# joeylitalien/drmlt-mitsuba

Measured on AMD Instinct MI355X. Metric: mutations/sec (accepted+rejected), higher is better.
Workload: dtype f32

## Files before the change

### drmlt-mitsuba_amd/csrc/device_sampler.h

```cpp
#pragma once
#include "device_math.h"
#include "device_types.h"

extern __shared__ __attribute__((aligned(16))) float lds_x[];

#define FP_STRICT _Pragma("clang fp contract(off)")

DEV float load_global_f32(const float *p) { return *(const float __attribute__((address_space(1))) *) (uintptr_t) p; }

enum { SM_BOOT = 0, SM_ARRAY = 1, SM_STAGE1 = 2, SM_STAGE2 = 3, SM_REVERSE = 4, SM_PT = 5 };

DEV float wrap01(float y) { return y > 1.f ? 2.f - y : fabsf(y); }
DEV float unwrap01(float v) { return v < 0.f ? 2.f - v : (v > 1.f ? -v : v); }

#define KELEMEN_S1 (1.0f / 1024.0f)
#define KELEMEN_S2 (1.0f / 64.0f)
#define ORBITAL_SCALE 1.9f
#define LOG2_S1_OVER_S2 (-4.0f)
#define WC_DISPERSION 0.96954361f

DEV float kelemen_sample(float xi, float s2) {
        FP_STRICT;
    float sign = 1.f;
    if (xi < 0.5f) { xi *= 2.f; } else { sign = -1.f; xi = 2.f * (xi - 0.5f); }
// ... 91 lines not shown
    uint32_t lane;
    uint32_t u1_off, s2_off;
    uint32_t stride;

    DEV void reset_caches() {}
    DEV float x(uint32_t k) const { return lds_x[k * stride + lane]; }
    DEV float u1(uint32_t k) const { return lds_x[u1_off + k * stride + lane]; }
    DEV float s2(uint32_t k) const { return lds_x[s2_off + k * stride + lane]; }
    DEV void put4(uint32_t off, const Unit4 &u) const {
        float *dst = &lds_x[off + lane];
        dst[0] = u.v[0]; dst[stride] = u.v[1]; dst[2u * stride] = u.v[2]; dst[3u * stride] = u.v[3];
    }

    DEV void fill_stage1(uint32_t b0, uint32_t b1) {
        for (uint32_t b = b0; b < b1; ++b) put4(u1_off + b * 4u * stride, philox_unit4(key0, key1, b, major, chain, TAG_S1));
    }
    DEV void fill_stage2(uint32_t D4, uint32_t first, uint32_t step) {
        if (large || type == 2) {
            const uint32_t rows = large ? D4 : (D4 / 2u + 3u) & ~3u;
            for (uint32_t b = first; b < rows / 4u; b += step) put4(s2_off + b * 4u * stride, philox_unit4(key0, key1, b, major, chain, TAG_S2));
        } else {
            for (uint32_t b = first; b < D4 / 2u; b += step) {
                const Unit4 u = philox_unit4(key0, key1, b, major, chain, TAG_S2);
                float *dst = &lds_x[s2_off + b * 2u * stride + lane];
                dst[0] = gaussian_sample(u.v[0], u.v[1], sigma2);
                dst[stride] = gaussian_sample(u.v[2], u.v[3], sigma2);
            }
        }
    }

    DEV float y_raw(uint32_t k) const {
        if (large) return u1(k);
        if (type != 2) return iid_first(u1(k), x(k));
        const uint32_t k0 = k & ~1u;
        return orbital_first(u1(k0), u1(k0 + 1u), (k & 1u) != 0u, x(k));
    }
    DEV float z_raw(uint32_t k) const {
        if (large) return s2(k);
        if (type != 2) return iid_second(x(k), s2(k));
        float z0, z1;
        orbital_pair(k & ~1u, true, z0, z1);
        return (k & 1u) ? z1 : z0;
    }
    DEV float next(uint32_t k) const {
        if (type == 2 && mode == SM_STAGE1) {
            const uint32_t k0 = k & ~1u;
            const bool odd = (k & 1u) != 0u;
            const float ua = u1(k0), ub = u1(k0 + 1u);
            const float y = orbital_first(ua, ub, odd, x(k));
            return wrap01(large ? (odd ? ub : ua) : y);
        }
        if (type == 2) {
            float z0, z1;
            orbital_pair(k & ~1u, true, z0, z1);
            const float zl = s2(k);
            return wrap01(large ? zl : ((k & 1u) ? z1 : z0));
        }
        const float xk = x(k), a = u1(k), g = s2(k);
        const float y = large ? a : iid_first(a, xk);
        const float z = large ? g : iid_second(xk, g);
        const float v = mode == SM_STAGE1 ? y : (mode == SM_STAGE2 ? z : green_reverse(xk, y, z));
        return wrap01(v);
    }
    DEV void orbital_pair(uint32_t k0, bool second, float &o0, float &o1) const {
        const float x0 = x(k0), x1 = x(k0 + 1u);
        float y0, y1;
        orbital_first_pair(u1(k0), u1(k0 + 1u), x0, x1, y0, y1);
        if (!second) { o0 = y0; o1 = y1; return; }
        orbital_second_pair(s2(k0 >> 1), x0, x1, y0, y1, o0, o1);
    }
};

template <int RULE = RULE_GENERIC> struct RowSamplerT {
    static constexpr bool orbital = RULE == RULE_ORBITAL;
    static constexpr bool batch_draws = true;
    uint32_t key0, key1;
    int mode, type;
    float sigma2;
    uint32_t stride, x_off, y_off, xyz;

    DEV void reset_caches() {}
    DEV float x(uint32_t k) const { return wrap01(lds_x[x_off + k * stride]); }
    DEV float y_raw(uint32_t k) const { return lds_x[y_off + k * stride]; }
    DEV uint32_t z_off() const { return xyz - x_off - y_off; }
    DEV float z_raw(uint32_t k) const { return lds_x[z_off() + k * stride]; }
    DEV float next(uint32_t k) const {
        if constexpr (orbital) return wrap01(lds_x[(mode == SM_STAGE1 ? y_off : z_off()) + k * stride]);
        float v = y_raw(k);
        if (mode != SM_STAGE1) {
            const float z = z_raw(k);
            v = mode == SM_STAGE2 ? z : green_reverse(x(k), v, z);
        }
        return wrap01(v);
    }
    DEV void adopt(int commit_mode) {
        const uint32_t xo = x_off, zo = z_off();
        x_off = commit_mode == SM_STAGE1 ? y_off : (commit_mode == SM_STAGE2 ? zo : xo);
        y_off = commit_mode == SM_STAGE1 ? xo : y_off;
    }
    DEV uint32_t roles() const { return (x_off << 1) | (y_off << 16); }
    DEV void set_roles(uint32_t w, uint32_t group, uint32_t col) { x_off = (w >> 1) & 0x7fffu; y_off = w >> 16; xyz = 3u * (group + col); }
    DEV static uint32_t first_roles(uint32_t group, uint32_t col) { return (col << 1) | ((group + col) << 16); }
    DEV void fill_first(uint32_t b, uint32_t major, uint32_t chain, bool large) const {
        const Unit4 u = philox_unit4(key0, key1, b, major, chain, TAG_S1);
        const float *xs = &lds_x[x_off + 4u * b * stride];
        float *ys = &lds_x[y_off + 4u * b * stride];
        const float x4[4] = {wrap01(xs[0]), wrap01(xs[stride]), wrap01(xs[2u * stride]), wrap01(xs[3u * stride])};
        float y[4];
        first_stage_block(orbital ? 2 : type, large, u, x4, y);
        ys[0] = y[0]; ys[stride] = y[1]; ys[2u * stride] = y[2]; ys[3u * stride] = y[3];
    }
    DEV void fill_second(uint32_t b, uint32_t D4, uint32_t major, uint32_t chain, bool large) const {
        const uint32_t nblk = large ? D4 / 4u : ((orbital || type == 2) ? (D4 / 2u + 3u) / 4u : D4 / 2u);
        if (b >= nblk) return;
        const Unit4 u = philox_unit4(key0, key1, b, major, chain, TAG_S2);
        const uint32_t zo = z_off();
        if (large) {
#pragma unroll
            for (uint32_t i = 0; i < 4u; ++i) lds_x[zo + (4u * b + i) * stride] = u.v[i];
        } else if (orbital || type == 2) {
            float xa[4], xb[4], ya[4], yb[4];
#pragma unroll
            for (uint32_t i = 0; i < 4u; ++i) {
                const uint32_t k0 = 2u * (4u * b + i), kk = k0 + 1u < D4 ? k0 : 0u;
                xa[i] = x(kk); xb[i] = x(kk + 1u);
                ya[i] = y_raw(kk); yb[i] = y_raw(kk + 1u);
            }
#pragma unroll
            for (uint32_t i = 0; i < 4u; ++i) {
                const uint32_t k0 = 2u * (4u * b + i);
                if (k0 + 1u < D4) {
                    float z0, z1;
                    orbital_second_pair(u.v[i], xa[i], xb[i], ya[i], yb[i], z0, z1);
                    lds_x[zo + k0 * stride] = z0;
                    lds_x[zo + (k0 + 1u) * stride] = z1;
                }
            }
        } else {
            const uint32_t k = 2u * b;
            const float x0 = x(k), x1 = x(k + 1u);
            lds_x[zo + k * stride] = iid_second(u.v[0], u.v[1], sigma2, x0);
            lds_x[zo + (k + 1u) * stride] = iid_second(u.v[2], u.v[3], sigma2, x1);
        }
    }
};
typedef RowSamplerT<> RowSampler;
template <int RULE> DEV void row_fill_first_drawn(const RowSamplerT<RULE> &s, uint32_t b, const Unit4 &u, bool large) {
    const float *xs = &lds_x[s.x_off + 4u * b * s.stride];
    float *ys = &lds_x[s.y_off + 4u * b * s.stride];
    const float x4[4] = {wrap01(xs[0]), wrap01(xs[s.stride]), wrap01(xs[2u * s.stride]), wrap01(xs[3u * s.stride])};
    float y[4];
    first_stage_block(RowSamplerT<RULE>::orbital ? 2 : s.type, large, u, x4, y);
    ys[0] = y[0]; ys[s.stride] = y[1]; ys[2u * s.stride] = y[2]; ys[3u * s.stride] = y[3];
}

struct RowsLds {
    DEV float get(uint32_t k, uint32_t col) const { return lds_x[k * 64u + col]; }
    DEV void put(uint32_t k, uint32_t col, float v) const { lds_x[k * 64u + col] = v; }
};
struct RowsMem {
    typedef float __attribute__((address_space(1))) *GPtr;
    GPtr base;
    uint32_t stride;
    DEV float get(uint32_t k, uint32_t col) const { return base[(size_t) k * stride + col]; }
    DEV void put(uint32_t k, uint32_t col, float v) const { base[(size_t) k * stride + col] = v; }
};

template <class Rows> struct PoolRowSampler {
    static constexpr bool batch_draws = true;
    uint32_t lane;
    Rows rows;
    const float *mira_x = nullptr;
    size_t mira_stride = 0;
    uint32_t mira_k0 = 0u, mira_k1 = 0u, mira_major = 0u, mira_chain = 0u, cached = 0xffffffffu;
    u4 blk = {0u, 0u, 0u, 0u};
    DEV void reset_caches() { cached = 0xffffffffu; }
    DEV float row(uint32_t k) const { return rows.get(k, lane); }
    DEV float next(uint32_t k) const { return wrap01(row(k)); }
    DEV float x(uint32_t k) const { return load_global_f32(mira_x + (size_t) k * mira_stride); }
    DEV float y_raw(uint32_t k) {
        if (cached != (k >> 2)) { cached = k >> 2; blk = philox4x32_10(mira_k0, mira_k1, cached, mira_major, mira_chain, TAG_S1); }
        uint32_t bx = blk.x, by = blk.y, bz = blk.z, bw = blk.w;
        asm volatile("" : "+v"(bx), "+v"(by), "+v"(bz), "+v"(bw));
        const uint32_t c = k & 3u, w = (c & 2u) ? ((c & 1u) ? bw : bz) : ((c & 1u) ? by : bx);
        return iid_first(u32_to_unit(w), x(k));
    }
    DEV float z_raw(uint32_t k) const { return row(k); }
};

struct State4 { float x0, x1, x2, x3; };
DEV State4 v5_state4(const DParams &P, uint32_t D, size_t xcol, uint32_t b) {
    const bool hi = 4u * b + 2u < D;
    const float *xs = P.x + (size_t) (4u * b) * P.n_chains + xcol;
    State4 X;
    X.x0 = load_global_f32(xs); X.x1 = load_global_f32(xs + P.n_chains);
    X.x2 = load_global_f32(xs + (hi ? 2u : 0u) * (size_t) P.n_chains); X.x3 = load_global_f32(xs + (hi ? 3u : 1u) * (size_t) P.n_chains);
    return X;
}
template <class Rows> DEV void v5_fill_first(const DParams &P, const Rows &rows, uint32_t D, uint32_t col, const State4 &X, uint32_t b, uint32_t major, uint32_t chain, bool large) {
    const Unit4 u = philox_unit4(P.key0, P.key1, b, major, chain, TAG_S1);
    const float u0 = u.v[0], u1 = u.v[1], u2 = u.v[2], u3 = u.v[3];
    const bool hi = 4u * b + 2u < D;
    const float x0 = X.x0, x1 = X.x1, x2 = X.x2, x3 = X.x3;
    float y0, y1, y2, y3;
    if (P.type == 2) {
        orbital_first_pair(u0, u1, x0, x1, y0, y1);
        orbital_first_pair(u2, u3, x2, x3, y2, y3);
    } else {
        y0 = iid_first(u0, x0); y1 = iid_first(u1, x1);
        y2 = iid_first(u2, x2); y3 = iid_first(u3, x3);
    }
    rows.put(4u * b, col, large ? u0 : y0); rows.put(4u * b + 1u, col, large ? u1 : y1);
    if (hi) { rows.put(4u * b + 2u, col, large ? u2 : y2); rows.put(4u * b + 3u, col, large ? u3 : y3); }
}
template <class Rows> DEV void v5_fill_second(const DParams &P, const Rows &rows, uint32_t D, uint32_t col, size_t xcol, uint32_t b, uint32_t major, uint32_t chain, bool large) {
    const Unit4 u = philox_unit4(P.key0, P.key1, b, major, chain, TAG_S2);
    if (large) {
#pragma unroll
        for (uint32_t i = 0; i < 4u; ++i)
            if (4u * b + i < D) rows.put(4u * b + i, col, u.v[i]);
        return;
    }
    if (P.type != 2) {
        const uint32_t k = 2u * b;
        const float x0 = load_global_f32(P.x + (size_t) k * P.n_chains + xcol), x1 = load_global_f32(P.x + (size_t) (k + 1u) * P.n_chains + xcol);
        rows.put(k, col, iid_second(u.v[0], u.v[1], P.sigma2, x0));
        rows.put(k + 1u, col, iid_second(u.v[2], u.v[3], P.sigma2, x1));
        return;
    }
    float xa[4], xb[4], ya[4], yb[4];
#pragma unroll
    for (uint32_t i = 0; i < 4u; ++i) {
        const uint32_t k0 = 2u * (4u * b + i);
        const uint32_t kk = k0 + 1u < D ? k0 : 0u;
        xa[i] = load_global_f32(P.x + (size_t) kk * P.n_chains + xcol); xb[i] = load_global_f32(P.x + (size_t) (kk + 1u) * P.n_chains + xcol);
        ya[i] = rows.get(kk, col); yb[i] = rows.get(kk + 1u, col);
    }
#pragma unroll
    for (uint32_t i = 0; i < 4u; ++i) {
        const uint32_t k0 = 2u * (4u * b + i);
        if (k0 + 1u < D) {
            float z0, z1;
            orbital_second_pair(u.v[i], xa[i], xb[i], ya[i], yb[i], z0, z1);
            rows.put(k0, col, z0);
            rows.put(k0 + 1u, col, z1);
        }
    }
}
template <class Rows> DEV void v5_iid_second_again(const DParams &P, const Rows &rows, uint32_t D, uint32_t col, size_t xcol, uint32_t b, uint32_t major, uint32_t chain, bool large, bool reverse) {
    const Unit4 u2 = philox_unit4(P.key0, P.key1, b, major, chain, TAG_S2);
    if (large) {
        Unit4 u1 = u2;
        if (reverse) u1 = philox_unit4(P.key0, P.key1, b, major, chain, TAG_S1);
#pragma unroll
        for (uint32_t i = 0; i < 4u; ++i) {
            const uint32_t k = 4u * b + i;
            if (k < D) {
                float *xg = P.x + (size_t) k * P.n_chains + xcol;
                if (reverse) rows.put(k, col, green_reverse(load_global_f32(xg), u1.v[i], u2.v[i]));
                else *xg = wrap01(u2.v[i]);
            }
        }
        return;
    }
    const uint32_t k = 2u * b;
    float *xg0 = P.x + (size_t) k * P.n_chains + xcol, *xg1 = xg0 + P.n_chains;
    const float x0 = load_global_f32(xg0), x1 = load_global_f32(xg1);
    const float z0 = iid_second(u2.v[0], u2.v[1], P.sigma2, x0), z1 = iid_second(u2.v[2], u2.v[3], P.sigma2, x1);
    if (!reverse) { *xg0 = wrap01(z0); *xg1 = wrap01(z1); return; }
    const u4 r1 = philox4x32_10(P.key0, P.key1, k >> 2, major, chain, TAG_S1);
    const float ua = (k & 2u) ? u32_to_unit(r1.z) : u32_to_unit(r1.x), ub = (k & 2u) ? u32_to_unit(r1.w) : u32_to_unit(r1.y);
    const float y0 = iid_first(ua, x0), y1 = iid_first(ub, x1);
    rows.put(k, col, green_reverse(x0, y0, z0));
    rows.put(k + 1u, col, green_reverse(x1, y1, z1));
}

struct PssmltSampler {
    uint32_t key0, key1, chain, major;
    bool large, kelemen;
    float sigma;
    uint32_t lane;
    uint32_t n_exist;
    u4 b1;
    uint32_t b1_idx;
    DEV void reset_caches() { b1_idx = 0xffffffffu; }
    DEV float u_s1(uint32_t idx) {
        uint32_t blk = idx >> 2;
        if (blk != b1_idx) { b1 = philox4x32_10(key0, key1, blk, major, chain, TAG_S1); b1_idx = blk; }
        return pick4(b1, idx & 3u);
    }
    DEV float x(uint32_t k) const { return lds_x[k * 64u + lane]; }
    DEV float next(uint32_t k) {
        const uint32_t per = (large || kelemen) ? 1u : 2u;
        if (k >= n_exist) return u_s1(per * n_exist + (k - n_exist));
        if (large) return u_s1(k);
        float value = x(k);
        if (kelemen) {
            float xi = u_s1(k);
            const bool add = xi < 0.5f;
            xi = add ? 2.f * xi : 2.f * (xi - 0.5f);
            const float dv = KELEMEN_S2 * fast_exp2(xi * LOG2_S1_OVER_S2);
            if (add) { value += dv; if (value > 1.f) value -= 1.f; }
            else { value -= dv; if (value < 0.f) value += 1.f; }
            return value;
        }
        const float v = value + gaussian_sample(u_s1(2u * k), u_s1(2u * k + 1u), sigma);
// ... 4 lines not shown
```

### drmlt-mitsuba_amd/csrc/kernels.hip

```cpp
#include <algorithm>
#include <cstdlib>
#include <cstdio>
#include <type_traits>
#include "device_path.h"

#include "kernel_common.h"
#include "launch_plan.h"

__device__ __attribute__((noinline)) DSplat eval_boot_sample(const DParams &P, uint32_t index, uint32_t &nd) {
    Sampler smp;
    smp.key0 = P.key0; smp.key1 = P.key1; smp.chain = P.boot_stream; smp.major = index;
    smp.mode = SM_BOOT; smp.arr = nullptr;
    uint32_t nr;
    return eval_path(P, smp, nr, nd);
}

__global__ void __launch_bounds__(64) k_bootstrap(DParams P, uint32_t n, float *lum_out) {
    uint32_t i = blockIdx.x * blockDim.x + threadIdx.x;
    if (i >= n) return;
    uint32_t nd;
    DSplat s = eval_boot_sample(P, i, nd);
    lum_out[i] = s.lum;
    if (P.boot_weighted) { normalize_splat(s, P); lum_out[(size_t) n + i] = s.lum; }
}
// ... 890 lines not shown
    G.z0 = v[8]; G.z1 = v[9]; G.z2 = v[10]; G.z3 = v[11];
}
DEV W2HeldScene w2_held_scene(const DParams &P) {
    W2HeldScene H;
    const uint32_t n_box = (uint32_t) min(max(P.n_box, 0), 3), n_flat = (uint32_t) min(max(P.n_flat_rec, 0), 1);
#pragma unroll
    for (uint32_t i = 0; i < 3u; ++i) {
        BoxRec &G = H.S.box[i];
        const DPrimBox *q = P.prims_box + i;
        w2_hold_rows(G, q->c, q->rz, i < n_box);
        uint32_t f0 = 0u, f1 = 0u, f2 = 0u;
        if (i < n_box) { f0 = q->fw[0]; f1 = q->fw[1]; f2 = q->fw[2]; }
        hold_v(f0); hold_v(f1); hold_v(f2);
        G.f0 = f0; G.f1 = f1; G.f2 = f2;
    }
    FlatRec &F = H.S.flat;
    w2_hold_rows(F, P.prims_flat->c, P.prims_flat->rz, n_flat > 0u);
    int ks = -1;
    if (n_flat > 0u) ks = P.prims_flat->kind_shade;
    hold_v(ks);
    F.ks = ks;
    H.counts = n_box | (n_flat << 8);
    hold_v(H.counts);
    return H;
}

template <bool HELD> __global__ void __launch_bounds__(CHAIN_BLOCK, 2) k_mutate_w2(DParams P, uint32_t n_mut, uint32_t mut_base) {
    typedef RowSamplerT<RULE_ORBITAL> RowSampler;
    if (threadIdx.x == 0) {
        atomicAdd(P.stats + 14, 1ull); atomicAdd(P.stats + 15, 1ull); atomicAdd(P.stats + 16, 1ull);
        if constexpr (HELD) atomicAdd(P.stats + 17, 1ull);
    }
    const uint32_t lane = threadIdx.x;
    const uint32_t sub = lane & 31u;
    const bool helper = lane >= 32u;
    const uint32_t c = blockIdx.x * 32u + sub;
    const bool live = !helper && c < P.n_chains;
    const uint32_t cc = c < P.n_chains ? c : P.n_chains - 1;
    const uint32_t S = V4_STRIDE;
    int smp_mode = SM_STAGE1;
    uint32_t roles;
    uint32_t qn = 0u;
    ChainState cs;
    float cum = 0.f;
    Counters ct = {0u, 0u, 0u, 0u, 0u};
    PathState ps;
    bool helper_has_ray = false;
    Hit h{-1, 0.f, 0.f, 0.f};
    int batch;
    uint32_t base = 0u, target = 0u, limit = 0u;
    bool reported = false;
    W2Held held = w2_held(P);
    w2_hold(held);
    typename std::conditional<HELD, W2HeldScene, W2StreamedScene>::type scene;
    if constexpr (HELD) scene = w2_held_scene(P);
    uint32_t imp_lo = (uint32_t) (uintptr_t) P.importance, imp_hi = (uint32_t) ((uintptr_t) P.importance >> 32);
    uint32_t done_lo = (uint32_t) (uintptr_t) P.chain_done, done_hi = (uint32_t) ((uintptr_t) P.chain_done >> 32);
    uint32_t left_lo = (uint32_t) (uintptr_t) P.waves_left, left_hi = (uint32_t) ((uintptr_t) P.waves_left >> 32);
    uint32_t key0_v = P.key0, key1_v = P.key1, chain_off_v = P.chain_offset, timid_v = (uint32_t) P.timid_after_large;
    hold_v(imp_lo); hold_v(imp_hi); hold_v(done_lo); hold_v(done_hi); hold_v(left_lo); hold_v(left_hi);
    hold_v(key0_v); hold_v(key1_v); hold_v(chain_off_v); hold_v(timid_v);
    {
        const V4Layout<RULE_ORBITAL> Y = v4_layout<RULE_ORBITAL>(P, V4_QCAP);
        roles = RowSampler::first_roles(Y.group, sub);
        if (!helper) {
            for (uint32_t k = 0; k < Y.D; ++k) lds_x[k * S + sub] = unwrap01(P.x[(size_t) k * P.n_chains + cc]);
            for (uint32_t k = Y.D; k < Y.D4; ++k) lds_x[k * S + sub] = 0.f;
        }
        cs.cur.lum = P.cur_lum[cc]; cs.cur.px = P.cur_px[cc]; cs.cur.py = P.cur_py[cc];
        cs.cur.r = P.cur_r[cc]; cs.cur.g = P.cur_g[cc]; cs.cur.b = P.cur_b[cc];
        cs.y = cs.cur; cs.z = cs.cur;
        cs.a1 = 0.f; cs.coin_acc1 = cs.coin_acc2 = cs.coin_mix = 0.f;
        cs.it = 0u; cs.nd1 = cs.nd2 = 0u; cs.stage = -1; cs.large = false;
        path_init(P, ps);
        base = (P.chain_done && live) ? P.chain_done[cc] : mut_base;
        target = P.chain_done ? n_mut : mut_base + n_mut;
        limit = P.chain_done ? P.run_limit : target;
        ps.phase = (live && base < limit) ? PH_DONE : PH_IDLE;
        ps.o = mk3(0.f, 0.f, 0.f); ps.d = mk3(0.f, 0.f, 1.f); ps.tmin = 0.f; ps.tmax = 0.f;
        batch = P.mh_batch > 32 ? 32 : P.mh_batch;
        stage_tables(P, Y.LT, lane);
        if (!helper) {
            const u4 coins = philox4x32_10(P.key0, P.key1, 0u, base, P.chain_offset + blockIdx.x * 32u + sub, TAG_COIN);
            float *dst = &lds_x[Y.L.coin_off + sub];
            dst[0] = u32_to_unit(coins.x); dst[S] = u32_to_unit(coins.y); dst[2u * S] = u32_to_unit(coins.z); dst[3u * S] = u32_to_unit(coins.w);
        }
    }

    for (;;) {
        const bool parked = ps.phase == PH_DONE;
        const unsigned long long pmask = __ballot(parked);
        const unsigned long long rmask = __ballot(ps.phase != PH_DONE && ps.phase != PH_IDLE);
        if (!pmask && !rmask) break;
        if (pmask && (__popcll(pmask) >= batch || !rmask)) {
            DParams Pm{};
            Pm.importance = uniform_ptr<const float>(imp_lo, imp_hi); Pm.width = (int) wave_uniform((uint32_t) held.width); Pm.height = (int) wave_uniform((uint32_t) held.height);
            Pm.chain_done = uniform_ptr<uint32_t>(done_lo, done_hi); Pm.waves_left = uniform_ptr<uint32_t>(left_lo, left_hi);
            Pm.key0 = wave_uniform(key0_v); Pm.key1 = wave_uniform(key1_v); Pm.chain_offset = wave_uniform(chain_off_v);
            Pm.eff_dim = (int) wave_uniform((uint32_t) held.eff_dim); Pm.timid_after_large = (int) wave_uniform(timid_v);
            Pm.use_mixture = 0; Pm.acceptance_map = 0; Pm.type = 2;
            const W2Held &C = held;
            const V4Lds L{C.coin_off, C.list_off, C.q_off, C.qcap};
            RowSampler smp = w2_sampler(Pm.key0, Pm.key1);
            smp.set_roles(roles, C.group, sub); smp.mode = smp_mode;
            const uint32_t D4 = ((uint32_t) Pm.eff_dim + 3u) & ~3u, nb1 = D4 / 4u;
            int *const lds_list = reinterpret_cast<int *>(&lds_x[L.list_off]);
            __builtin_amdgcn_s_setprio(2);
            if (qn + 64u > wave_uniform(L.qcap)) { SECTION_PARAMS(Pf); w2_flush(Pf, L, qn, lane); }
            int commit = 0, kind = 0;
            W2hQueued qa{false, 0.f, 0.f, 0.f, 0.f, 0.f}, qb{false, 0.f, 0.f, 0.f, 0.f, 0.f};
            if constexpr (HELD) w2h_decide(Pm, parked, cs, ps, ct, cum, commit, kind, qa, qb);
            else if (parked) {
                const MhDigest o = mh_decide<RULE_ORBITAL>(Pm, cs, smp, ps, ct);
                if (o.decided) {
                    cum += o.w.w0;
                    const bool a1st = o.acc1, a2nd = o.acc2, adopt = a1st || a2nd;
                    const DSplat sb = select_splat(a2nd, cs.y, cs.z);
                    const float wb = a2nd ? o.w.w1 : o.w.w2;
                    qb.want = !a1st && wb > 0.f;
                    qb.px = sb.px; qb.py = sb.py; qb.r = sb.r * wb; qb.g = sb.g * wb; qb.b = sb.b * wb;
                    const DSplat sa = select_splat(adopt, cs.cur, cs.y);
                    const float wa = adopt ? cum : o.w.w1;
                    qa.want = wa > 0.f;
                    qa.px = sa.px; qa.py = sa.py; qa.r = sa.r * wa; qa.g = sa.g * wa; qa.b = sa.b * wa;
                    if (adopt) {
                        cum = a1st ? o.w.w1 : o.w.w2;
                        cs.cur = select_splat(a1st, cs.y, cs.z);
                    }
                    commit = mh_commit_mode(o);
                }
                kind = cs.stage < 0 ? 4 : 2;
            }
            kind = mh_resolve_kind(Pm, kind, live, base + cs.it, target, limit, reported, lane);
            v4_enqueue(L, qn, qa.want, qa.px, qa.py, qa.r, qa.g, qa.b);
            v4_enqueue(L, qn, qb.want, qb.px, qb.py, qb.r, qb.g, qb.b);


            smp.adopt(commit);
            roles = smp.roles();

            if (parked && kind == 1) {
                const float *cn = &lds_x[L.coin_off + sub];
                cs.large = cn[0] < C.p_large;
                cs.coin_acc1 = cn[S]; cs.coin_acc2 = cn[2u * S]; cs.coin_mix = cn[3u * S];
                cs.stage = 0;
                cs.nd1 = cs.nd2 = 0u;
            }

            RowSampler smg = w2_sampler(Pm.key0, Pm.key1);
            const uint32_t chain_base_g = Pm.chain_offset + blockIdx.x * 32u;
            const uint32_t maj_mine = base + cs.it;
            const unsigned info = roles | (cs.large ? 1u : 0u);
            const uint32_t f1mask = (uint32_t) __ballot(kind == 1);
            if (f1mask) {
                if (kind == 1) lds_list[__builtin_amdgcn_mbcnt_lo(f1mask, 0u)] = (int) sub;
                const uint32_t n = (uint32_t) __popc(f1mask), total = n * (nb1 + 1u);
                const float rcp_n = 1.f / (float) n;
                for (uint32_t fb = 0u; fb < total; fb += 64u) {
                    const uint32_t i = fb + lane;
                    const bool valid = i < total;
                    const uint32_t ii = valid ? i : 0u;
                    const uint32_t b = (uint32_t) (((float) ii + 0.5f) * rcp_n), j = ii - b * n;
                    const uint32_t cj = (uint32_t) lds_list[j];
                    const uint32_t mj = (uint32_t) __shfl((int) maj_mine, (int) cj, 64);
                    const unsigned inf = (unsigned) __shfl((int) info, (int) cj, 64);
                    smg.set_roles(inf, C.group, cj);
                    const bool coin = b >= nb1;
                    if (valid) {
                        const u4 r = philox4x32_10(Pm.key0, Pm.key1, coin ? 0u : b, coin ? mj + 1u : mj, chain_base_g + cj, coin ? TAG_COIN : TAG_S1);
                        const Unit4 u{{u32_to_unit(r.x), u32_to_unit(r.y), u32_to_unit(r.z), u32_to_unit(r.w)}};
                        if (!coin) row_fill_first_drawn(smg, b, u, (inf & 1u) != 0u);
                        else {
                            float *dst = &lds_x[L.coin_off + cj];
                            dst[0] = u.v[0]; dst[S] = u.v[1]; dst[2u * S] = u.v[2]; dst[3u * S] = u.v[3];
                        }
                    }
                }
            }
            const uint32_t f2mask = (uint32_t) __ballot(kind == 2);
            if (f2mask) {
                if (kind == 2) lds_list[__builtin_amdgcn_mbcnt_lo(f2mask, 0u)] = (int) sub;
                const uint32_t nb2 = Pm.timid_after_large ? D4 / 4u : (D4 / 2u + 3u) / 4u;
                const uint32_t n = (uint32_t) __popc(f2mask), total = n * nb2;
                const float rcp_n = 1.f / (float) n;
                for (uint32_t fb = 0u; fb < total; fb += 64u) {
                    const uint32_t i = fb + lane;
                    const bool valid = i < total;
                    const uint32_t ii = valid ? i : 0u;
                    const uint32_t b = (uint32_t) (((float) ii + 0.5f) * rcp_n), j = ii - b * n;
                    const uint32_t cj = (uint32_t) lds_list[j];
                    const uint32_t mj = (uint32_t) __shfl((int) maj_mine, (int) cj, 64);
                    const unsigned inf = (unsigned) __shfl((int) info, (int) cj, 64);
                    smg.set_roles(inf, C.group, cj);
                    if (valid) smg.fill_second(b, D4, mj, chain_base_g + cj, (inf & 1u) != 0u);
                }
            }

            if (parked) {
                if (kind == 0) ps.phase = PH_IDLE;
                else {
                    DParams Vb{};
                    Vb.exclude_direct = C.exclude_direct; Vb.width = C.width; Vb.height = C.height;
                    Vb.tan_half_fov = C.tan_half_fov; Vb.inv_aspect = C.inv_aspect; Vb.near_clip = C.near_clip; Vb.far_clip = C.far_clip;
#pragma unroll
                    for (int q = 0; q < 12; ++q) Vb.cam[q] = C.cam[q];
                    smp_mode = smp.mode = cs.stage == 0 ? SM_STAGE1 : SM_STAGE2;
                    path_init(Vb, ps);
                    const float v0 = smp.next(0u), v1 = smp.next(1u);
                    path_begin(Vb, ps, v0, v1);
                }
            }
        }
        const bool tracing = helper ? helper_has_ray : ps.phase == PH_CLOSEST;
        __builtin_amdgcn_s_setprio(0);
        if constexpr (HELD) {
            if (__ballot(tracing)) {
                const uint32_t counts = wave_uniform(scene.counts);
                h = trace_held(scene.S, counts & 0xffu, counts >> 8, ps.o, ps.d, ps.tmin, ps.tmax);
            }
        } else {
            SECTION_PARAMS(Pt);
            if (__ballot(tracing)) h = trace<0>(Pt, ps.o, ps.d, ps.tmin, ps.tmax, helper);
        }
        __builtin_amdgcn_s_setprio(3);
        const unsigned occluded = from_upper_u((helper_has_ray && h.prim >= 0) ? 1u : 0u);
        helper_has_ray = false;
        ShadowRay sr;
        asm volatile("" : "=v"(sr.d.x), "=v"(sr.d.y), "=v"(sr.d.z), "=v"(sr.tmin), "=v"(sr.tmax));
        sr.o = ps.o; sr.valid = false;
        {
            const W2Held &Cs = held;
            if (!helper && ps.phase != PH_DONE && ps.phase != PH_IDLE) {
                RowSampler sms = w2_sampler(0u, 0u);
                sms.set_roles(roles, Cs.group, sub); sms.mode = smp_mode;
                DParams Vs{};
                Vs.eff_dim = Cs.eff_dim; Vs.rr_depth = Cs.rr_depth; Vs.max_depth = Cs.max_depth;
                const LdsTables LT{Cs.shade_off, Cs.bsdf_off, 0u};
                path_step_diffuse<RowSampler, HeldLightTables, false, HELD>(Vs, HeldLightTables{LT, Cs.light, Cs.light_shade}, ps, sms, h, occluded == 0u, sr);
            }
        }
        ps.o.x = lower_keeps(ps.o.x, sr.o.x); ps.o.y = lower_keeps(ps.o.y, sr.o.y); ps.o.z = lower_keeps(ps.o.z, sr.o.z);
        ps.d.x = lower_keeps(ps.d.x, sr.d.x); ps.d.y = lower_keeps(ps.d.y, sr.d.y); ps.d.z = lower_keeps(ps.d.z, sr.d.z);
        ps.tmin = lower_keeps(ps.tmin, sr.tmin); ps.tmax = lower_keeps(ps.tmax, sr.tmax);
        helper_has_ray = lower_keeps_u(0u, sr.valid ? 1u : 0u) != 0u;
    }
    SECTION_PARAMS(Pe);
    const V4Layout<RULE_ORBITAL> Y = v4_layout<RULE_ORBITAL>(Pe, V4_QCAP);
    if (qn + 32u > Y.L.qcap) w2_flush(Pe, Y.L, qn, lane);
    v4_enqueue(Y.L, qn, live && cum > 0.f, cs.cur.px, cs.cur.py, cs.cur.r * cum, cs.cur.g * cum, cs.cur.b * cum);
    w2_flush(Pe, Y.L, qn, lane);
    if (live) {
        RowSampler smp = Y.smp;
        smp.set_roles(roles, Y.group, sub);
        for (uint32_t k = 0; k < Y.D; ++k) Pe.x[(size_t) k * Pe.n_chains + c] = smp.x(k);
        Pe.cur_lum[c] = cs.cur.lum; Pe.cur_px[c] = cs.cur.px; Pe.cur_py[c] = cs.cur.py;
        Pe.cur_r[c] = cs.cur.r; Pe.cur_g[c] = cs.cur.g; Pe.cur_b[c] = cs.cur.b;
        if (Pe.chain_done) Pe.chain_done[c] = base + cs.it;
    }
    if (Pe.chain_done && !reported && lane == 0) atomicSub(Pe.waves_left, 1u);
    flush_counters(Pe, ct, lane);
    const unsigned long long decided = wave_sum((live && !helper) ? cs.it : 0u);
    if (lane == 0) atomicAdd(Pe.stats + 9, decided);
}

#define V5_STACK32_CAP 25
#ifndef V5_ROWS_MEM_WAVES
#define V5_ROWS_MEM_WAVES 3
#endif
#ifndef V5_ROWS_MEM_STACK32_CAP
#define V5_ROWS_MEM_STACK32_CAP 25
#endif
enum { RS_IDLE = 0, RS_BUSY = 1, RS_DONE = 2 };

struct V5Lds {
    uint32_t coin_off, list_off;
    uint32_t q_off;
    uint32_t pool_off;
    uint32_t ring_off;
    uint32_t status_off;
};
DEV V5Lds v5_layout(uint32_t D, uint32_t qcap, bool coin_rows) {
    V5Lds L;
    L.coin_off = D * 64u;
    L.list_off = L.coin_off + (coin_rows ? 4u * 64u : 0u);
    L.q_off = L.list_off + 64u;
    L.pool_off = L.q_off + 5u * qcap;
    L.ring_off = L.pool_off + 8u * V5_SLOTS;
    L.status_off = L.ring_off + V5_SLOTS / 4u;
    return L;
}

template <int FEAT, bool STACK16, bool OVF, bool STAMPS = false, bool LDS_TABLES = false, bool ROWS_MEM = false>
__global__ void __launch_bounds__(CHAIN_BLOCK, ROWS_MEM ? V5_ROWS_MEM_WAVES : 2) k_mutate_v5(DParams P, uint32_t n_mut, uint32_t mut_base) {
    constexpr bool FLAT = (FEAT & 8) == 0;
    typedef typename std::conditional<ROWS_MEM, RowsMem, RowsLds>::type RowsT;
    typedef PoolRowSampler<RowsT> SamplerT;
    constexpr uint32_t QCAP = (FLAT || STACK16) ? V5_QCAP : V5_QCAP_STACK32;
    constexpr bool COIN_ROWS = FLAT || STACK16;
    SECTION_PARAMS(P0);
    const uint32_t lane = threadIdx.x;
    const uint32_t wave_base = blockIdx.x * 64u;
    const uint32_t c = wave_base + lane;
    const bool live = c < P0.n_chains;
    const uint32_t cc = live ? c : P0.n_chains - 1;
    const uint32_t D = (uint32_t) P0.eff_dim, nb1 = (D + 3u) / 4u;
    const V5Lds L = v5_layout(ROWS_MEM ? 0u : D, QCAP, COIN_ROWS);
    const V4Lds Lq{0u, 0u, L.q_off, QCAP};
    unsigned char *const ring = reinterpret_cast<unsigned char *>(&lds_x[L.ring_off]);
    unsigned char *const status = reinterpret_cast<unsigned char *>(&lds_x[L.status_off]);
    int *const lds_list = reinterpret_cast<int *>(&lds_x[L.list_off]);
    float *const pool = &lds_x[L.pool_off];
    status[lane] = RS_IDLE; status[64u + lane] = RS_IDLE;
    LdsTables LT;
    LT.shade_off = L.status_off + V5_SLOTS / 4u;
    LT.bsdf_off = LT.shade_off + (uint32_t) P0.n_shade * 16u;
    LT.emit_off = LT.bsdf_off + (uint32_t) P0.n_bsdfs * 12u;
    if (LDS_TABLES) stage_tables(P0, LT, lane);
    HybridTables HT;
    HT.L.shade_off = L.status_off + V5_SLOTS / 4u;
    HT.L.bsdf_off = HT.L.shade_off + (uint32_t) P0.n_emitters * 16u;
    HT.L.emit_off = HT.L.bsdf_off + (uint32_t) P0.n_bsdfs * 12u;
    HT.lds = !FLAT && P0.small_tables_lds != 0;
    if (HT.lds) stage_bsdfs_emitters(P0, HT.L, lane);

    ChainState cs;
    cs.cur.lum = P0.cur_lum[cc]; cs.cur.px = P0.cur_px[cc]; cs.cur.py = P0.cur_py[cc];
    cs.cur.r = P0.cur_r[cc]; cs.cur.g = P0.cur_g[cc]; cs.cur.b = P0.cur_b[cc];
    cs.y = cs.cur; cs.z = cs.cur;
    cs.a1 = 0.f; cs.coin_acc1 = cs.coin_acc2 = cs.coin_mix = 0.f;
    cs.it = 0u; cs.nd1 = cs.nd2 = 0u; cs.stage = -1; cs.large = false;
    float cum = 0.f;
    uint32_t qn = 0u;
    Counters ct = {0u, 0u, 0u, 0u, 0u};
    RowsT rows;
    if constexpr (ROWS_MEM) { rows.base = (RowsMem::GPtr) (uintptr_t) (P0.rows + wave_base); rows.stride = P0.n_chains; }
    SamplerT smp{lane, rows};

    PathState ps;
    path_init(P0, ps);
    ps.o = mk3(0.f, 0.f, 0.f); ps.d = mk3(0.f, 0.f, 1.f); ps.tmin = 0.f; ps.tmax = 0.f;
    const uint32_t base = (P0.chain_done && live) ? P0.chain_done[cc] : mut_base;
    const uint32_t target = P0.chain_done ? n_mut : mut_base + n_mut;
    const uint32_t limit = P0.chain_done ? P0.run_limit : target;
    bool reported = false;
    ps.phase = (live && base < limit) ? PH_DONE : PH_IDLE;
    const int batch = P0.mh_batch > 64 ? 64 : P0.mh_batch;
    if (COIN_ROWS) {
// ... 502 lines not shown
```

Before: 3.321 billion.

## Merge stage-one and stage-two row fills into one wave-wide loop for held chains

For the HELD template variant, the separate stage-one and stage-two row-fill loops are combined into a single loop over a joint work list. Each stage-two block is split across four lanes, each computing one orbital pair, which gives finer-grained work items. The goal is fewer idle lanes and fewer loop trips when both kinds of chains are present. In exchange each iteration carries more divergent select logic, uses asm barriers to pin values in registers, and stage-two lanes compute redundantly when a block is large.

```diff
diff --git a/drmlt-mitsuba_amd/csrc/device_sampler.h b/drmlt-mitsuba_amd/csrc/device_sampler.h
--- a/drmlt-mitsuba_amd/csrc/device_sampler.h
+++ b/drmlt-mitsuba_amd/csrc/device_sampler.h
@@ -267,6 +267,28 @@
     float y[4];
     first_stage_block(RowSamplerT<RULE>::orbital ? 2 : s.type, large, u, x4, y);
     ys[0] = y[0]; ys[s.stride] = y[1]; ys[2u * s.stride] = y[2]; ys[3u * s.stride] = y[3];
+}
+template <int RULE> DEV void row_fill_second_pair_drawn(const RowSamplerT<RULE> &s, uint32_t b, uint32_t p, uint32_t D4, const Unit4 &u, bool large) {
+    static_assert(RowSamplerT<RULE>::orbital, "the orbital arm of fill_second");
+    const uint32_t nblk = large ? D4 / 4u : (D4 / 2u + 3u) / 4u;
+    const uint32_t k0 = 2u * (4u * b + p), kk = k0 + 1u < D4 ? k0 : 0u;
+    float xa = lds_x[s.x_off + kk * s.stride], xb = lds_x[s.x_off + (kk + 1u) * s.stride];
+    float ya = s.y_raw(kk), yb = s.y_raw(kk + 1u);
+    asm volatile("" : "+v"(xa), "+v"(xb), "+v"(ya), "+v"(yb));
+    const bool hi = (p & 2u) != 0u, odd = (p & 1u) != 0u;
+    float u0 = u.v[0], u1 = u.v[1], u2 = u.v[2], u3 = u.v[3];
+    asm volatile("" : "+v"(u0), "+v"(u1), "+v"(u2), "+v"(u3));
+    const float xi = hi ? (odd ? u3 : u2) : (odd ? u1 : u0);
+    const float la = odd ? u2 : u0, lb = odd ? u3 : u1;
+    float z0, z1;
+    orbital_second_pair(xi, wrap01(xa), wrap01(xb), ya, yb, z0, z1);
+    asm volatile("" : "+v"(z0), "+v"(z1));
+    const bool put = b < nblk && (large ? !hi : k0 + 1u < D4);
+    const uint32_t zo = s.z_off(), row = large ? 4u * b + 2u * p : k0;
+    if (put) {
+        lds_x[zo + row * s.stride] = large ? la : z0;
+        lds_x[zo + (row + 1u) * s.stride] = large ? lb : z1;
+    }
 }
 
 struct RowsLds {
diff --git a/drmlt-mitsuba_amd/csrc/kernels.hip b/drmlt-mitsuba_amd/csrc/kernels.hip
--- a/drmlt-mitsuba_amd/csrc/kernels.hip
+++ b/drmlt-mitsuba_amd/csrc/kernels.hip
@@ -1066,47 +1066,84 @@
             const uint32_t maj_mine = base + cs.it;
             const unsigned info = roles | (cs.large ? 1u : 0u);
             const uint32_t f1mask = (uint32_t) __ballot(kind == 1);
-            if (f1mask) {
-                if (kind == 1) lds_list[__builtin_amdgcn_mbcnt_lo(f1mask, 0u)] = (int) sub;
-                const uint32_t n = (uint32_t) __popc(f1mask), total = n * (nb1 + 1u);
-                const float rcp_n = 1.f / (float) n;
-                for (uint32_t fb = 0u; fb < total; fb += 64u) {
-                    const uint32_t i = fb + lane;
-                    const bool valid = i < total;
-                    const uint32_t ii = valid ? i : 0u;
-                    const uint32_t b = (uint32_t) (((float) ii + 0.5f) * rcp_n), j = ii - b * n;
-                    const uint32_t cj = (uint32_t) lds_list[j];
-                    const uint32_t mj = (uint32_t) __shfl((int) maj_mine, (int) cj, 64);
-                    const unsigned inf = (unsigned) __shfl((int) info, (int) cj, 64);
-                    smg.set_roles(inf, C.group, cj);
-                    const bool coin = b >= nb1;
-                    if (valid) {
-                        const u4 r = philox4x32_10(Pm.key0, Pm.key1, coin ? 0u : b, coin ? mj + 1u : mj, chain_base_g + cj, coin ? TAG_COIN : TAG_S1);
-                        const Unit4 u{{u32_to_unit(r.x), u32_to_unit(r.y), u32_to_unit(r.z), u32_to_unit(r.w)}};
-                        if (!coin) row_fill_first_drawn(smg, b, u, (inf & 1u) != 0u);
-                        else {
-                            float *dst = &lds_x[L.coin_off + cj];
-                            dst[0] = u.v[0]; dst[S] = u.v[1]; dst[2u * S] = u.v[2]; dst[3u * S] = u.v[3];
+            if constexpr (HELD) {
+                const uint32_t f2mask = (uint32_t) __ballot(kind == 2);
+                if (f1mask | f2mask) {
+                    const uint32_t n1 = (uint32_t) __popc(f1mask), n2 = (uint32_t) __popc(f2mask);
+                    if (kind == 1 || kind == 2) lds_list[kind == 1 ? __builtin_amdgcn_mbcnt_lo(f1mask, 0u) : n1 + __builtin_amdgcn_mbcnt_lo(f2mask, 0u)] = (int) sub;
+                    const uint32_t nb2 = Pm.timid_after_large ? D4 / 4u : (D4 / 2u + 3u) / 4u;
+                    const uint32_t t1 = n1 * (nb1 + 1u), total = t1 + n2 * 4u * nb2;
+                    for (uint32_t fb = 0u; fb < total; fb += 64u) {
+                        const uint32_t i = fb + lane;
+                        const bool valid = i < total, second = valid && i >= t1;
+                        const uint32_t ii = valid ? (second ? i - t1 : i) : 0u, n = second ? n2 : n1;
+                        const uint32_t q = (uint32_t) (((float) ii + 0.5f) * __builtin_amdgcn_rcpf((float) n)), j = ii - q * n;
+                        const uint32_t b = second ? q >> 2 : q;
+                        const uint32_t cj = (uint32_t) lds_list[second ? n1 + j : j];
+                        const uint32_t mj = (uint32_t) __shfl((int) maj_mine, (int) cj, 64);
+                        const unsigned inf = (unsigned) __shfl((int) info, (int) cj, 64);
+                        smg.set_roles(inf, C.group, cj);
+                        const bool coin = !second && b >= nb1;
+                        Unit4 u{{0.f, 0.f, 0.f, 0.f}};
+                        if (valid) {
+                            const u4 r = philox4x32_10(Pm.key0, Pm.key1, coin ? 0u : b, coin ? mj + 1u : mj, chain_base_g + cj, coin ? TAG_COIN : (second ? TAG_S2 : TAG_S1));
+                            u = Unit4{{u32_to_unit(r.x), u32_to_unit(r.y), u32_to_unit(r.z), u32_to_unit(r.w)}};
+                            if (!second) {
+                                if (!coin) row_fill_first_drawn(smg, b, u, (inf & 1u) != 0u);
+                                else {
+                                    float *dst = &lds_x[L.coin_off + cj];
+                                    dst[0] = u.v[0]; dst[S] = u.v[1]; dst[2u * S] = u.v[2]; dst[3u * S] = u.v[3];
+                                }
+                            }
+                        }
+                        if (__ballot(second)) {
+                            if (second) row_fill_second_pair_drawn(smg, b, q & 3u, D4, u, (inf & 1u) != 0u);
                         }
                     }
                 }
-            }
-            const uint32_t f2mask = (uint32_t) __ballot(kind == 2);
-            if (f2mask) {
-                if (kind == 2) lds_list[__builtin_amdgcn_mbcnt_lo(f2mask, 0u)] = (int) sub;
-                const uint32_t nb2 = Pm.timid_after_large ? D4 / 4u : (D4 / 2u + 3u) / 4u;
-                const uint32_t n = (uint32_t) __popc(f2mask), total = n * nb2;
-                const float rcp_n = 1.f / (float) n;
-                for (uint32_t fb = 0u; fb < total; fb += 64u) {
-                    const uint32_t i = fb + lane;
-                    const bool valid = i < total;
-                    const uint32_t ii = valid ? i : 0u;
-                    const uint32_t b = (uint32_t) (((float) ii + 0.5f) * rcp_n), j = ii - b * n;
-                    const uint32_t cj = (uint32_t) lds_list[j];
-                    const uint32_t mj = (uint32_t) __shfl((int) maj_mine, (int) cj, 64);
-                    const unsigned inf = (unsigned) __shfl((int) info, (int) cj, 64);
-                    smg.set_roles(inf, C.group, cj);
-                    if (valid) smg.fill_second(b, D4, mj, chain_base_g + cj, (inf & 1u) != 0u);
+            } else {
+                if (f1mask) {
+                    if (kind == 1) lds_list[__builtin_amdgcn_mbcnt_lo(f1mask, 0u)] = (int) sub;
+                    const uint32_t n = (uint32_t) __popc(f1mask), total = n * (nb1 + 1u);
+                    const float rcp_n = 1.f / (float) n;
+                    for (uint32_t fb = 0u; fb < total; fb += 64u) {
+                        const uint32_t i = fb + lane;
+                        const bool valid = i < total;
+                        const uint32_t ii = valid ? i : 0u;
+                        const uint32_t b = (uint32_t) (((float) ii + 0.5f) * rcp_n), j = ii - b * n;
+                        const uint32_t cj = (uint32_t) lds_list[j];
+                        const uint32_t mj = (uint32_t) __shfl((int) maj_mine, (int) cj, 64);
+                        const unsigned inf = (unsigned) __shfl((int) info, (int) cj, 64);
+                        smg.set_roles(inf, C.group, cj);
+                        const bool coin = b >= nb1;
+                        if (valid) {
+                            const u4 r = philox4x32_10(Pm.key0, Pm.key1, coin ? 0u : b, coin ? mj + 1u : mj, chain_base_g + cj, coin ? TAG_COIN : TAG_S1);
+                            const Unit4 u{{u32_to_unit(r.x), u32_to_unit(r.y), u32_to_unit(r.z), u32_to_unit(r.w)}};
+                            if (!coin) row_fill_first_drawn(smg, b, u, (inf & 1u) != 0u);
+                            else {
+                                float *dst = &lds_x[L.coin_off + cj];
+                                dst[0] = u.v[0]; dst[S] = u.v[1]; dst[2u * S] = u.v[2]; dst[3u * S] = u.v[3];
+                            }
+                        }
+                    }
+                }
+                const uint32_t f2mask = (uint32_t) __ballot(kind == 2);
+                if (f2mask) {
+                    if (kind == 2) lds_list[__builtin_amdgcn_mbcnt_lo(f2mask, 0u)] = (int) sub;
+                    const uint32_t nb2 = Pm.timid_after_large ? D4 / 4u : (D4 / 2u + 3u) / 4u;
+                    const uint32_t n = (uint32_t) __popc(f2mask), total = n * nb2;
+                    const float rcp_n = 1.f / (float) n;
+                    for (uint32_t fb = 0u; fb < total; fb += 64u) {
+                        const uint32_t i = fb + lane;
+                        const bool valid = i < total;
+                        const uint32_t ii = valid ? i : 0u;
+                        const uint32_t b = (uint32_t) (((float) ii + 0.5f) * rcp_n), j = ii - b * n;
+                        const uint32_t cj = (uint32_t) lds_list[j];
+                        const uint32_t mj = (uint32_t) __shfl((int) maj_mine, (int) cj, 64);
+                        const unsigned inf = (unsigned) __shfl((int) info, (int) cj, 64);
+                        smg.set_roles(inf, C.group, cj);
+                        if (valid) smg.fill_second(b, D4, mj, chain_base_g + cj, (inf & 1u) != 0u);
+                    }
                 }
             }
 
```

After: 3.367 billion (median of 6 runs). +1.4%, better.
